# too-z/MultiModalPFN

Hardware: AMD Instinct MI355X
Metric: in-context rows/sec (support+query), PAD-UFES-20 shape, 1/2/4/8 MI355X (higher is better)
Workload: dtype f16

## Files before the change

### include/mmpfn_hip.h

```cpp
#ifndef MMPFN_HIP_H_
#define MMPFN_HIP_H_

#include <stdint.h>

#ifdef __cplusplus
extern "C" {
#endif

#define MMPFN_OK 0
#define MMPFN_ERR_INVALID (-1)
#define MMPFN_ERR_HIP (-2)
#define MMPFN_ERR_NAN (-3)
#define MMPFN_ERR_STATE (-4)
#define MMPFN_ERR_WEIGHT (-5)

#define MMPFN_PREC_F32 0
#define MMPFN_PREC_BF16 1
#define MMPFN_PREC_F32_MFMA 2
#define MMPFN_PREC_BF16_F8 3
#define MMPFN_PREC_BF16_F8E5 4
#define MMPFN_PREC_F16 5
#define MMPFN_PREC_F16_F8 6
#define MMPFN_PREC_F16_F8E5 7

// ... 30 lines not shown
const char* mmpfn_last_error(const mmpfn_ctx* ctx);
int mmpfn_set_stream(mmpfn_ctx* ctx, void* hip_stream);
const char* mmpfn_version(void);

int mmpfn_set_model(mmpfn_ctx* ctx, const mmpfn_model_desc* desc);
int mmpfn_load_weight(mmpfn_ctx* ctx, const char* name, const float* host_data, int64_t numel);
int mmpfn_finalize_weights(mmpfn_ctx* ctx);

int mmpfn_mixer_tokens(const mmpfn_ctx* ctx, int n_mod);
int mmpfn_mixer_forward(mmpfn_ctx* ctx, const float* image, int S, int n_mod, float* tokens, int precision);

int mmpfn_forward(mmpfn_ctx* ctx, const float* x, int S, int F, const float* tokens, int C, const float* y_train,
                  int N, const float* uniq, int U, const float* pos_rand, float* logits, int precision);

int mmpfn_set_full_last_layer(mmpfn_ctx* ctx, int on);

int mmpfn_embed(mmpfn_ctx* ctx, const float* x, int S, int F, const float* tokens, int C, const float* y_train, int N,
                const float* uniq, int U, const float* pos_rand, int precision);
int mmpfn_run_layers(mmpfn_ctx* ctx, int layer_begin, int layer_end);
int mmpfn_decode(mmpfn_ctx* ctx, float* logits);
int mmpfn_copy_state(mmpfn_ctx* ctx, float* out, int64_t capacity_elems);
int mmpfn_state_tokens(const mmpfn_ctx* ctx);

int mmpfn_aggregate(mmpfn_ctx* ctx, const float* logits, int M, int Q, int n_out, const int* perms, int n_cls,
                    float temperature, int average_before_softmax, const float* class_weights, float* probs);

#define MMPFN_BAR_MAX_BARS 8192
#define MMPFN_BAR_MAX_MEMBERS 1024
#define MMPFN_BAR_MAX_LEVELS 64
int mmpfn_bar_head(mmpfn_ctx* ctx, const float* logits, int M, int Q, int B, const unsigned char* cancel, int ldc,
// ... 71 lines not shown
```

### multimodalpfn_amd/_lib.py

```python

from __future__ import annotations

import ctypes
import os
from pathlib import Path

LIB_PATH = Path(__file__).resolve().parent / "libmmpfn_hip.so"

MMPFN_OK = 0
MMPFN_MAX_LANES = 8
MMPFN_ERR_INVALID = -1
MMPFN_ERR_HIP = -2
MMPFN_ERR_NAN = -3
MMPFN_ERR_STATE = -4
MMPFN_ERR_WEIGHT = -5
BAR_MAX_BARS, BAR_MAX_MEMBERS, BAR_MAX_LEVELS = 8192, 1024, 64
BAR_MAX_TARGETS, BAR_SCORE_ENDS = 64, 9

PREC_F32 = 0
PREC_BF16 = 1
PREC_F32_MFMA = 2
PREC_BF16_F8 = 3
PREC_BF16_F8E5 = 4
PREC_F16 = 5
# ... 83 lines not shown
    ("mmpfn_cache_free", None, [_vp, _vp]),
    ("mmpfn_kernel_timing", _i, [_vp, _i]),
    ("mmpfn_feature_attention", _i, [_vp, _i, _vp, _i, _i, _i]),
    ("mmpfn_feature_attention_ex", _i, [_vp, _i, _vp, _i, _i, _i, _i, _i]),
    ("mmpfn_item_attention_block", _i, [_vp, _i, _vp, _i, _i, _i, _i]),
    ("mmpfn_mlp_ln", _i, [_vp, _i, _vp, _i64, _i]),
    ("mmpfn_outproj_mlp_ln", _i, [_vp, _i, _vp, _vp, _i64, _i]),
    ("mmpfn_item_qkv", _i, [_vp, _i, _vp, _i, _i, _i, _i, _i, _i, _vp, _vp, _vp]),
    ("mmpfn_mgm", _i, [_vp, _vp, _i, _i, _vp, _i]),
    ("mmpfn_cap", _i, [_vp, _vp, _i, _i, _vp, _i]),
    ("mmpfn_kernel_timing_read", _i, [_vp, ctypes.POINTER(ctypes.c_double), ctypes.POINTER(ctypes.c_int64),
                                      ctypes.POINTER(ctypes.c_double)]),
    ("mmpfn_siphash24_rows", _i, [_vp, _i64, _i64, _vp]),
    ("mmpfn_set_parity_attention_min_keys", _i, [_i, _i]),
    ("mmpfn_set_full_last_layer", _i, [_vp, _i]),
    ("mmpfn_bar_head", _i, [_vp, _vp, _i, _i, _i, _vp, _i, _vp, _vp, _i, _f, _i, _vp, _vp, _vp, _vp, _vp, _i, _vp, _vp,
                            _vp, _vp]),
    ("mmpfn_bar_score", _i, [_vp, _vp, _i, _i, _f, _vp, _vp, _vp, _vp, _vp, _vp, _vp, _i, _vp, _vp, _vp, _vp, _vp]),
    ("mmpfn_bar_head_score", _i, [_vp, _vp, _i, _i, _i, _vp, _i, _vp, _vp, _i, _f, _i, _vp, _vp, _vp, _vp, _vp, _i, _vp,
                                  _vp, _vp, _vp, _vp, _vp, _vp, _vp, _vp, _i, _vp, _vp, _vp, _vp, _vp]),
]

MMPFN_ENC_VIT = 1
MMPFN_ENC_TEXT = 2


class EncDesc(ctypes.Structure):
    _fields_ = [
        ("kind", ctypes.c_int),
        ("dim", ctypes.c_int),
# ... 89 lines not shown
```

### multimodalpfn_amd/csrc/attention.hip

```cpp
#include <atomic>

#include "attn_item.h"
#include "common.h"
#include "kernels.h"

namespace mmpfn {

namespace {

constexpr int IA_KT = 64;

template <bool BF16>
struct IaLds {
  static constexpr int KROW = BF16 ? 80 : 144;
  static constexpr int VROW = BF16 ? 136 : 272;
  static constexpr int KBYTES = IA_KT * KROW;
  static constexpr int VBYTES = 32 * VROW;
  static constexpr int STAGE = KBYTES + VBYTES;
};

constexpr float IA_TAU = 8.0f;

template <int MODE, int NW>
__global__ __launch_bounds__(64 * NW) void attn_item_kernel(const AttnArgs p) {
// ... 696 lines not shown
      exact_rows(p, Kg, Vg, qrow, orow, qok[qb] && hh == 0, c);
      continue;
    }
    const float inv = 1.0f / ls;
    if (qok[qb]) {
#pragma unroll
      for (int gq = 0; gq < 4; ++gq)
        *(f32x4*)(orow + 8 * gq + 4 * hh) = f32x4{o[qb][4 * gq] * inv, o[qb][4 * gq + 1] * inv,
                                                  o[qb][4 * gq + 2] * inv, o[qb][4 * gq + 3] * inv};
    }
  }
}

}


namespace {
#ifndef X3_CHEAP_MIN_KEYS
#define X3_CHEAP_MIN_KEYS (-1)
#endif
#ifndef X3_CHEAP_FORM
#define X3_CHEAP_FORM 3
#endif
std::atomic<int> g_x3_cheap_min_keys{X3_CHEAP_MIN_KEYS};
std::atomic<int> g_x3_cheap_form{X3_CHEAP_FORM};

hipError_t launch_item_attention(const AttnLayerArgs& l, bool x3, hipStream_t st) {
  const int T = l.T, H = l.H, Npad = l.Npad, nk = l.nk, na = l.na, nb = l.nb, kvb = l.kvb;
  if (na + nb <= 0 || T <= 0) return hipSuccess;
  if (nk <= 0 || Npad % A2_KT != 0 || nk > Npad || H > 8 || H <= 0) return hipErrorInvalidValue;
  if (nb > 0 && (kvb < 0 || kvb >= H)) return hipErrorInvalidValue;
  if (l.qk_t == DType::F32 || l.o_t == DType::F32 || (l.qk_t == DType::F16 && l.o_t != DType::F16))
    return hipErrorInvalidValue;
  Attn2Args a;
  a.q = (const bf16*)l.q, a.k = (const bf16*)l.k, a.vt = (const bf16*)l.vt, a.o = (bf16*)l.out;
  a.S = l.S, a.H = H, a.Npad = Npad, a.nk = nk;
  a.a0 = l.a0, a.na = na, a.b0 = l.b0, a.nb = nb, a.kvb = nb > 0 ? kvb : -1;
  a.kv_bstride = l.kv_bstride > 0 ? l.kv_bstride : (int64_t)H * Npad * 32;
  a.q_prescaled = !x3 && l.q_prescaled ? 1 : 0;
  a.vt8 = (const unsigned char*)l.vt8, a.f8 = x3 ? 0 : l.f8;
  a.qk_f16 = (!x3 && l.qk_t == DType::F16) ? 1 : 0;
  a.o_f16 = (!x3 && l.o_t == DType::F16) ? 1 : 0;
  if (l.kv_bstride > 0 && (na > 0 || kvb != 0)) return hipErrorInvalidValue;
  const int qpb = x3 ? A3_QPB : ATTN_ITEM_QPB;
  int acc = 0;
  for (int g = 0; g < H; ++g) {
    a.tstart[g] = acc;
    const int cnt = na + (g == a.kvb ? H * nb : 0);
    acc += (cnt + qpb - 1) / qpb;
  }
  for (int g = H; g < 9; ++g) a.tstart[g] = acc;
  a.tasks_per_b = acc;
  a.nblocks = acc * T;
  if (a.nblocks == 0) return hipSuccess;
  if (x3) {
    const int mk = g_x3_cheap_min_keys.load(std::memory_order_relaxed);
    const int form = mk >= 0 && nk >= mk ? g_x3_cheap_form.load(std::memory_order_relaxed) : 0;
    if (form == 1) hipLaunchKernelGGL(attn_item3_kernel<1>, dim3(a.nblocks), dim3(256), 0, st, a);
    else if (form == 2) hipLaunchKernelGGL(attn_item3_kernel<2>, dim3(a.nblocks), dim3(256), 0, st, a);
    else if (form == 3) hipLaunchKernelGGL(attn_item3_kernel<3>, dim3(a.nblocks), dim3(256), 0, st, a);
    else hipLaunchKernelGGL(attn_item3_kernel<0>, dim3(a.nblocks), dim3(256), 0, st, a);
    return hipGetLastError();
  }
  return launch_attn_pipe(a, st);
}

}

// ... 55 lines not shown
```

### multimodalpfn_amd/csrc/attention_pipe.hip

```cpp
#include <type_traits>

#include "attn_item.h"
#include "common.h"
#include "kernels.h"
#include "lds_dma.h"

namespace mmpfn {

namespace {

#ifdef MMPFN_STAMPS
constexpr int AP_NST = 48;
__device__ unsigned long long g_ap_stamps[8 * 4 * AP_NST];
__device__ int g_ap_meta[4];
#define AP_STAMP(k)                                                                                     \
  do {                                                                                                  \
    const int sb_ = (int)blockIdx.x - (int)(gridDim.x / 2);                                            \
    if (sb_ >= 0 && sb_ < 8 && lane == 0) g_ap_stamps[(sb_ * 4 + wave) * AP_NST + (k)] = __builtin_amdgcn_s_memtime(); \
  } while (0)
#elif defined(MMPFN_STAMPS_ALL)
constexpr int AP_NST = 36, AP_MAXB = 8192;
__device__ unsigned long long g_ap_all[AP_MAXB * 4 * (AP_NST + 2)];
#define AP_STAMP(k)                                                                                     \
  do {                                                                                                  \
// ... 31 lines not shown
template <> struct P8<2> {
  static constexpr int FMT = 1, ETOP = 6, EMIN = -16, EMAX = 15;
  static constexpr float UFLOW = 0x1p-10f;
  static __device__ __forceinline__ s16x2 cvt(s16x2 old, float a, float b, float sc, bool hi) {
    return hi ? __builtin_amdgcn_cvt_scalef32_pk_bf8_f32(old, a, b, sc, true)
              : __builtin_amdgcn_cvt_scalef32_pk_bf8_f32(old, a, b, sc, false);
  }
};

constexpr int SG_VALU = 0x2, SG_MFMA = 0x8, SG_VMEM_READ = 0x20, SG_DS_READ = 0x100, SG_DS_WRITE = 0x200,
              SG_TRANS = 0x400;

#ifndef P4_DMA
#define P4_DMA 1
#endif
template <int F8, bool QF16, bool OF16>
__global__ __launch_bounds__(256, 2) void attn_pipe_kernel(const Attn2Args p) {
  typedef typename Op16<QF16>::t QT;
  typedef typename Op16<QF16>::x8 Q8;
  typedef typename Op16<OF16>::t OT;
  typedef typename Op16<OF16>::x4 O4;
  constexpr bool DMA = F8 == 0 && P4_DMA;
  constexpr int KROW = DMA ? 64 : 80;
  constexpr int VROW = F8 ? 80 : (DMA ? 128 : 144);
  constexpr int P4_SLOT_BYTES = 64 * KROW + 32 * VROW;
  __shared__ __attribute__((aligned(1024))) unsigned char ring[4 * P4_SLOT_BYTES];
  const int tid = threadIdx.x, lane = tid & 63;
  const int wave = __builtin_amdgcn_readfirstlane(tid >> 6);
  const int r = lane & 31, hh = lane >> 5;
  AP_STAMP(0);
#ifdef MMPFN_STAMPS_ALL
  if (lane == 0 && blockIdx.x < AP_MAXB) {
    const size_t b0 = ((size_t)blockIdx.x * 4 + wave) * (AP_NST + 2);
    g_ap_all[b0] = __builtin_amdgcn_s_getreg(4 | (31 << 11));
    g_ap_all[b0 + 1] = __builtin_amdgcn_s_getreg(20 | (31 << 11));
  }
#endif

  int b, g, chunk;
  {
    const int task = xcd_task(blockIdx.x, p.nblocks);
    b = task / p.tasks_per_b;
    const int rem = task - b * p.tasks_per_b;
    g = 0;
    int base = p.tstart[0];
#pragma unroll
    for (int h = 1; h < 9; ++h)
      if (h < p.H && p.tstart[h] <= rem) g = h, base = p.tstart[h];
    chunk = rem - base;
  }
  const int cnt = item_count(p, g);
  const int jw = chunk * P4_QPB + wave * P4_QPW;
  const bool active = jw < cnt;

  const int64_t kvoff = (int64_t)b * p.kv_bstride + (int64_t)g * p.Npad * 32;
  const QT* Kg = (const QT*)p.k + kvoff;
  const bf16* Vg = p.vt + kvoff;
  const unsigned char* Vg8 = p.vt8 + kvoff;
  const float c = kLog2e * 0.17677669529663687f;

  auto qrow_of = [&](int qb) __attribute__((always_inline)) { return item_query(p, g, cnt, jw + 32 * qb + r); };
  Q8 qf[P4_NCH][2];
#pragma unroll
  for (int qb = 0; qb < P4_NCH; ++qb) {
    const ItemQuery q = qrow_of(qb);
    const QT* qrow = (const QT*)p.q + (((int64_t)b * p.H + q.h) * p.S + q.s) * 32;
#pragma unroll
// ... 42 lines not shown
  };
  using VFrag = std::conditional_t<F8 != 0, i32x8, bf16x8[2][2]>;
  using PFrag = std::conditional_t<F8 != 0, i32x8, bf16x8[2][2]>;
  using VStage = std::conditional_t<F8 != 0, u32x2, u32x4>;
  auto readv = [&](VFrag& vf, const unsigned char* slot) __attribute__((always_inline)) {
    if constexpr (F8 != 0) {
      const u32x4 a = *(const u32x4*)(slot + vb), c = *(const u32x4*)(slot + vb + 16);
      vf = i32x8{(int)a.x, (int)a.y, (int)a.z, (int)a.w, (int)c.x, (int)c.y, (int)c.z, (int)c.w};
    } else {
#pragma unroll
      for (int u = 0; u < 2; ++u)
#pragma unroll
        for (int sp = 0; sp < 2; ++sp) vf[u][sp] = *(const bf16x8*)(slot + vro[u][sp]);
    }
  };
  const int krow = tid >> 2, kc = tid & 3, vd = tid >> 3, vc = tid & 7;
  const int kso = krow * 32 + kc * 8, vso = vd * p.Npad + vc * 8;
  const int kw = krow * KROW + 16 * (DMA ? kc ^ ((krow >> 2) & 3) : kc);
  const int vw = F8    ? VBASE + vd * VROW + 32 * (vc & 1) + 8 * (vc >> 1)
                 : DMA ? VBASE + vd * VROW + 16 * (vc ^ ((vd >> 1) & 7))
                       : VBASE + vd * VROW + 16 * vc;
  uint32_t kdo = 0, vdo = 0;
  if constexpr (DMA) {
    const int R = 16 * wave + (lane >> 2), d = 8 * wave + (lane >> 3);
    kdo = (uint32_t)(R * 32 + 8 * ((lane & 3) ^ ((R >> 2) & 3))) * 2;
    vdo = (uint32_t)(d * p.Npad + 8 * ((lane & 7) ^ ((d >> 1) & 7))) * 2;
  }
  const unsigned lds0 = (unsigned)(uintptr_t)(__attribute__((address_space(3))) void*)ring;
  auto dma = [&](int t, int slot) __attribute__((always_inline)) {
    lds_dma16(kdo, Kg + (int64_t)t * (P4_KT * 32), __builtin_amdgcn_readfirstlane(lds0 + slot * P4_SLOT_BYTES + wave * 1024));
    lds_dma16(vdo, Vg + t * P4_KT,
             __builtin_amdgcn_readfirstlane(lds0 + slot * P4_SLOT_BYTES + VBASE + wave * 1024));
  };
#ifndef P4_LEAD
#define P4_LEAD 2
#endif
  constexpr int LEAD = P4_LEAD;
  static_assert(LEAD == 1 || LEAD == 2, "staging lead");
  u32x4 rk[LEAD];
  VStage rv[LEAD];
  auto gload = [&](int t, u32x4& k, VStage& v) __attribute__((always_inline)) {
    k = *(const u32x4*)(Kg + (int64_t)t * (P4_KT * 32) + kso);
    if constexpr (F8 != 0) v = *(const u32x2*)(Vg8 + t * P4_KT + vso);
    else v = *(const u32x4*)(Vg + t * P4_KT + vso);
  };
  auto lstore = [&](unsigned char* slot, const u32x4& k, const VStage& v) __attribute__((always_inline)) {
    *(u32x4*)(slot + kw) = k;
    *(VStage*)(slot + vw) = v;
  };
  auto mask_pad = [&](u32x4& k, VStage& v) {
    const int k0 = nfull * P4_KT;
    if (k0 + krow >= p.nk) k = u32x4{0u, 0u, 0u, 0u};
    if constexpr (F8 != 0) {
      uint64_t e = __builtin_bit_cast(uint64_t, v);
#pragma unroll
      for (int j = 0; j < 8; ++j)
        if (k0 + vc * 8 + j >= p.nk) e &= ~((uint64_t)0xff << (8 * j));
      v = __builtin_bit_cast(u32x2, e);
    } else {
      bf16x8 e = __builtin_bit_cast(bf16x8, v);
#pragma unroll
      for (int j = 0; j < 8; ++j)
        if (k0 + vc * 8 + j >= p.nk) e[j] = (bf16)0.0f;
      v = __builtin_bit_cast(u32x4, e);
    }
// ... 159 lines not shown
    }
    __builtin_amdgcn_sched_group_barrier(SG_TRANS, P4_PIN == 2 ? 8 : 4, 0);
    __builtin_amdgcn_sched_group_barrier(SG_VALU, 16, 0);
    if (mem && !DMA) {
      __builtin_amdgcn_sched_group_barrier(SG_DS_WRITE, 2, 0);
      __builtin_amdgcn_sched_group_barrier(SG_VMEM_READ, 2, 0);
    }
#endif
  };

  if (ntiles > 0) {
    Q8 kf[2][2][2];
    VFrag vf[2];
    f32x16 sa[2], sb[2];
    PFrag pa, pz;
    {
      u32x4 rk1;
      VStage rv1;
      gload(tile_of(0), rk[0], rv[0]);
      gload(tile_of(min(1, ntiles - 1)), rk1, rv1);
      if constexpr (DMA) dma(tile_of(min(2, ntiles - 1)), 2);
      if (partial) mask_pad(rk[0], rv[0]);
      lstore(ring, rk[0], rv[0]);
      lstore(ring + P4_SLOT_BYTES, rk1, rv1);
    }
    if constexpr (!DMA) {
      gload(tile_of(min(2, ntiles - 1)), rk[0], rv[0]);
      if constexpr (LEAD == 2) gload(tile_of(min(3, ntiles - 1)), rk[1], rv[1]);
    }
    lds_barrier();
    AP_STAMP(2);
    if (!active) {
      if constexpr (DMA) {
        for (int t = 0; t < ntiles; ++t) {
          dma(tile_of(min(t + 3, ntiles - 1)), (t + 3) & 3);
          lds_barrier();
        }
        __builtin_amdgcn_s_waitcnt(0x0070);
        return;
      }
      for (int t = 0; t < ntiles; t += LEAD) {
        lstore(ring + ((t + 2) & 3) * P4_SLOT_BYTES, rk[0], rv[0]);
        gload(tile_of(min(t + 2 + LEAD, ntiles - 1)), rk[0], rv[0]);
        lds_barrier();
        if (LEAD == 2 && t + 1 < ntiles) {
          lstore(ring + ((t + 3) & 3) * P4_SLOT_BYTES, rk[LEAD - 1], rv[LEAD - 1]);
          gload(tile_of(min(t + 5, ntiles - 1)), rk[LEAD - 1], rv[LEAD - 1]);
// ... 2 lines not shown
      }
      return;
    }
    readk(kf[0], ring);
    if constexpr (F8 != 0) {
      vf[0] = i32x8{0, 0, 0, 0, 0, 0, 0, 0}, pz = vf[0];
    } else {
#pragma unroll
      for (int u = 0; u < 2; ++u)
#pragma unroll
        for (int sp = 0; sp < 2; ++sp)
#pragma unroll
          for (int j = 0; j < 8; ++j) vf[0][u][sp][j] = pz[u][sp][j] = (bf16)0.0f;
    }
    smm(sa, kf[0], 0);
    if constexpr (F8 != 0) {
      f32x16 s1[2];
      smm(s1, kf[0], 1);
      const int k0 = tile_of(0) * P4_KT;
#pragma unroll
      for (int qb = 0; qb < P4_NCH; ++qb) {
        const f32x16(&s)[2] = qb == 0 ? sa : s1;
        float m = -INFINITY;
#pragma unroll
        for (int u = 0; u < 2; ++u)
#pragma unroll
          for (int i = 0; i < 16; ++i)
            if (k0 + 32 * u + 16 * (i >> 3) + 8 * hh + (i & 7) < p.nk) m = fmaxf(m, s[u][i]);
        const auto sw = __builtin_amdgcn_permlane32_swap(__float_as_uint(m), __float_as_uint(m), false, false);
        m = fmaxf(__uint_as_float(sw[0]), __uint_as_float(sw[1]));
// ... 25 lines not shown
      pin_step(true);
      if constexpr (DMA) dma(tile_of(min(t + 3, ntiles - 1)), (L + 3) & 3);
      smm(sa, kf[B], 0);
      expc(pz, sb, 1);
      pv(0, pa, vf[B]);
      pin_step(false);
      lds_barrier();
#if defined(MMPFN_STAMPS) || defined(MMPFN_STAMPS_ALL)
      if (t < AP_NST - 6) AP_STAMP(3 + t);
#endif
    };
    using I0 = std::integral_constant<int, 0>;
    using I1 = std::integral_constant<int, 1>;
    using I2 = std::integral_constant<int, 2>;
    using I3 = std::integral_constant<int, 3>;
    int t = 0;
    for (; t + 4 <= ntiles; t += 4) {
      iter(I0{}, t);
      iter(I1{}, t + 1);
      iter(I2{}, t + 2);
      iter(I3{}, t + 3);
    }
    if (t < ntiles) iter(I0{}, t++);
    if (t < ntiles) iter(I1{}, t++);
    if (t < ntiles) iter(I2{}, t++);
    if (ntiles & 1) pv(1, pz, vf[1]);
    else pv(1, pz, vf[0]);
  }
  AP_STAMP(AP_NST - 3);

  if (!active) return;
  float mref[P4_NCH] = {0.f, 0.f};
  auto tile1 = [&](int t, bool first, bool ref) {
    const int k0 = t * P4_KT;
    Q8 kf[2][2];
    bf16x8 vf[2][2];
    loadk(kf, t);
    loadv(vf, t);
    const bool mask = k0 + P4_KT > p.nk;
    if (mask) {
// ... 71 lines not shown
    for (int gq = 0; gq < 4; ++gq) {
      O4 v;
#pragma unroll
      for (int e = 0; e < 4; ++e) v[e] = (OT)(o[qb][4 * gq + e] * inv);
      w[gq] = __builtin_bit_cast(u32x2, v);
    }
#pragma unroll
    for (int gg = 0; gg < 4; gg += 2) {
      const auto sx = __builtin_amdgcn_permlane32_swap(w[gg].x, w[gg + 1].x, false, false);
      const auto sy = __builtin_amdgcn_permlane32_swap(w[gg].y, w[gg + 1].y, false, false);
      const u32x4 st = hh == 0 ? u32x4{w[gg].x, w[gg].y, sx[1], sy[1]} : u32x4{sx[0], sy[0], w[gg + 1].x, w[gg + 1].y};
      if (q.ok) *(u32x4*)(orow + 8 * gg + 8 * hh) = st;
    }
  }
  AP_STAMP(AP_NST - 1);
}

}

namespace {
template <bool QF16, bool OF16>
hipError_t launch_pipe(const Attn2Args& a, hipStream_t st) {
  if (a.f8 == 1) {
    if (!a.vt8) return hipErrorInvalidValue;
    hipLaunchKernelGGL((attn_pipe_kernel<1, QF16, OF16>), dim3(a.nblocks), dim3(256), 0, st, a);
  } else if (a.f8 == 2) {
    if (!a.vt8) return hipErrorInvalidValue;
    hipLaunchKernelGGL((attn_pipe_kernel<2, QF16, OF16>), dim3(a.nblocks), dim3(256), 0, st, a);
  } else {
    hipLaunchKernelGGL((attn_pipe_kernel<0, QF16, OF16>), dim3(a.nblocks), dim3(256), 0, st, a);
// ... 6 lines not shown
extern "C" int mmpfn_dbg_attn_stamps(unsigned long long* stamps, int* meta) {
  hipError_t e = hipMemcpyFromSymbol(stamps, HIP_SYMBOL(g_ap_stamps), sizeof(g_ap_stamps));
  if (e == hipSuccess) e = hipMemcpyFromSymbol(meta, HIP_SYMBOL(g_ap_meta), sizeof(g_ap_meta));
  return (int)e;
}
#endif

#ifdef MMPFN_STAMPS_ALL
extern "C" int mmpfn_dbg_attn_stamps_all(unsigned long long* out, int nblocks) {
  const size_t n = (size_t)(nblocks < AP_MAXB ? nblocks : AP_MAXB) * 4 * (AP_NST + 2) * sizeof(unsigned long long);
  return (int)hipMemcpyFromSymbol(out, HIP_SYMBOL(g_ap_all), n);
}
#endif

hipError_t launch_attn_pipe(const Attn2Args& a, hipStream_t st) {
  if (a.qk_f16) return launch_pipe<true, true>(a, st);
  return a.o_f16 ? launch_pipe<false, true>(a, st) : launch_pipe<false, false>(a, st);
}

namespace {
__global__ void vt_fp8_kernel(const u32x4* __restrict__ in, u32x2* __restrict__ out, int64_t n8) {
  const int64_t i = (int64_t)blockIdx.x * blockDim.x + threadIdx.x;
  if (i >= n8) return;
  const bf16x8 v = __builtin_bit_cast(bf16x8, in[i]);
  float f[8];
#pragma unroll
  for (int j = 0; j < 8; ++j) f[j] = fminf(fmaxf((float)v[j], -448.f), 448.f);
  s16x2 lo = __builtin_amdgcn_cvt_scalef32_pk_fp8_f32(s16x2{0, 0}, f[0], f[1], 1.0f, false);
  lo = __builtin_amdgcn_cvt_scalef32_pk_fp8_f32(lo, f[2], f[3], 1.0f, true);
  s16x2 hi = __builtin_amdgcn_cvt_scalef32_pk_fp8_f32(s16x2{0, 0}, f[4], f[5], 1.0f, false);
// ... 16 lines not shown
```

### multimodalpfn_amd/csrc/attn_item.h

```cpp
#pragma once
#include "common.h"
#include "kernels.h"

namespace mmpfn {

struct Attn2Args {
  const __bf16* q;
  const __bf16* k;
  const __bf16* vt;
  __bf16* o;
  int S, H, Npad, nk;
  int a0, na;
  int b0, nb, kvb;
  int tasks_per_b, nblocks;
  int tstart[9];
  int64_t kv_bstride;
  int q_prescaled;
  const unsigned char* vt8;
  int f8;
  int qk_f16;
  int o_f16;
};
hipError_t launch_attn_pipe(const Attn2Args& a, hipStream_t st);

__device__ __forceinline__ int item_count(const Attn2Args& p, int g) { return p.na + (g == p.kvb ? p.H * p.nb : 0); }

struct ItemQuery {
  int h, s;
  bool ok;
};
// ... 45 lines not shown
```

### multimodalpfn_amd/csrc/capi.cpp

```cpp
#include <hip/hip_runtime.h>

#include <cmath>
#include <cstdlib>
#include <cstdio>
#include <cstring>
#include <map>
#include <string>
#include <utility>
#include <vector>

#include "../../include/mmpfn_hip.h"
#include "devbuf.h"
#include "kernels.h"
#include "weight_pack.h"

using namespace mmpfn;

namespace {

struct LayerW {
  Weight feat_qkv, feat_out, item_qkv, item_qtest, item_out, mlp1, mlp2;
  Weight feat_pack;
};

// ... 35 lines not shown
  std::string err;
  bool have_model = false, finalized = false;
  mmpfn_model_desc d{};
  std::map<std::string, std::vector<float>> host;

  ModelWeights w;

  DevBuf mx[8];
  DevBuf tap_v8;
  DevBuf tap_x16;
  std::vector<Lane> lanes;
  int cur = 0;
  mmpfn_cache* cache_out = nullptr;
  const mmpfn_cache* cache_in = nullptr;
  bool full_last = false;
  bool kt_on = false;
  std::vector<hipEvent_t> kt_pool;
  size_t kt_used = 0;
  double kt_flops = 0.0;
};

namespace {

#define HIPCHK(expr) HIPCHK_ON(ctx, expr)
#define GETW(var, name, n) GETW_ON(ctx, var, name, n)

bool mgm_f16_shape(const mmpfn_model_desc& d) { return (d.mgm_heads * d.nhid) % 256 == 0; }

int ensure_flag(mmpfn_ctx* ctx, DevBuf& b, hipStream_t st) {
  if (b.p) return MMPFN_OK;
// ... 383 lines not shown
  const int eb = pm.op_bytes();
  hipStream_t st = ctx->stream;
  void* O = ctx->ws_O.p;
  unsigned char* big = (unsigned char*)ctx->ws_big.p;
  void* Qi = big;
  void* Ki = big + (size_t)RM * E * eb;
  void* Vi = (unsigned char*)Ki + (size_t)TM * H * Npad * 32 * eb;
  RC(item_project(ctx, l, Xv, S, T, N, Npad, M, pm, last, ctx->cache_in != nullptr, Qi, Ki, Vi));
  if (ctx->cache_in) {
    const mmpfn_cache* cc = ctx->cache_in;
    const size_t kvl = (size_t)T * cc->Npad * 32 * eb;
    const size_t ccol = (size_t)c0 * cc->Npad * 32 * eb;
    const unsigned char* Kc = (const unsigned char*)cc->kv.p + (size_t)l * 2 * kvl + ccol;
    AttnLayerArgs a{Qi, Kc, Kc + kvl, O, S, TM, H, cc->Npad, cc->N};
    a.a0 = 0, a.na = 0, a.b0 = 0, a.nb = S, a.kvb = 0;
    a.kv_bstride = (int64_t)cc->Npad * 32;
    a.q_prescaled = pm.is16(), a.qk_t = pm.qk(), a.o_t = pm.attn_out();
    HIPCHK(launch_attn_layer(a, pm.base, st));
  } else {
    if (ctx->cache_out) {
      mmpfn_cache* cc = ctx->cache_out;
      const size_t blk = (size_t)Npad * 32 * eb, kvl = (size_t)T * blk;
      unsigned char* Kc = (unsigned char*)cc->kv.p + (size_t)l * 2 * kvl + c0 * blk;
      HIPCHK(hipMemcpy2DAsync(Kc, blk, Ki, (size_t)H * blk, blk, nc, hipMemcpyDeviceToDevice, st));
      HIPCHK(hipMemcpy2DAsync(Kc + kvl, blk, Vi, (size_t)H * blk, blk, nc, hipMemcpyDeviceToDevice, st));
    }
    if (last && Q == 0) return MMPFN_OK;
    AttnLayerArgs a{Qi, Ki, Vi, O, S, TM, H, Npad, N};
    a.a0 = 0, a.na = N, a.b0 = N, a.nb = Q, a.kvb = 0;
    if (last) a.na = N % ATTN_ITEM_QPB, a.a0 = N - a.na;
    a.q_prescaled = pm.is16(), a.qk_t = pm.qk(), a.o_t = pm.attn_out();
    hipEvent_t* ev = nullptr;
    if (pm.is16()) {
      if (ctx->kt_on && !last) {
        if (ctx->kt_used + 2 > ctx->kt_pool.size()) {
          for (int i = 0; i < 64; ++i) {
            hipEvent_t e;
            HIPCHK(hipEventCreate(&e));
            ctx->kt_pool.push_back(e);
          }
        }
        ev = &ctx->kt_pool[ctx->kt_used];
        ctx->kt_used += 2;
        ctx->kt_flops += 4.0 * TM * (double)(N + Q) * N * E;
      }
// ... 535 lines not shown
    }
  }
  if (bad) return fail(ctx, MMPFN_ERR_NAN, "There should be no NaNs in the encoded x and y (flag " + std::to_string(bad) + ")");
  return MMPFN_OK;
}

static int attn_tap_args(mmpfn_ctx* ctx, const void* q, const void* k, const void* vt, void* out, int S, int T, int H,
                         int Hmax, int Npad, int nk, int a0, int na, int b0, int nb, int kvb, AttnLayerArgs& a) {
  if (!ctx || !q || !k || !vt || !out) return MMPFN_ERR_INVALID;
  if (a0 < 0 || na < 0 || a0 + na > S || b0 < 0 || nb < 0 || b0 + nb > S || nk <= 0 || nk > Npad || Npad % 64 ||
      H <= 0 || H > Hmax || T <= 0 || kvb >= H)
    return fail(ctx, MMPFN_ERR_INVALID, "bad attention geometry");
  HIPCHK(hipSetDevice(ctx->device));
  a = AttnLayerArgs{q, k, vt, out, S, T, H, Npad, nk};
  a.a0 = a0, a.na = na, a.b0 = b0, a.nb = nb, a.kvb = kvb;
  return MMPFN_OK;
}

int mmpfn_item_attention(mmpfn_ctx* ctx, const void* q, const void* k, const void* vt, void* out, int S, int T, int H,
                         int Npad, int s0, int nq, int nk, int kvh, int precision) {
  AttnLayerArgs a;
  if (kvh < 0) RC(attn_tap_args(ctx, q, k, vt, out, S, T, H, INT32_MAX, Npad, nk, s0, nq, 0, 0, -1, a));
  else RC(attn_tap_args(ctx, q, k, vt, out, S, T, H, INT32_MAX, Npad, nk, 0, 0, s0, nq, kvh, a));
  if (precision != PREC_F32 && precision != PREC_BF16 && precision != PREC_F32_MFMA)
    return fail(ctx, MMPFN_ERR_INVALID, "bad precision (PREC_F32, PREC_BF16 or PREC_F32_MFMA; 16-bit / fp8 Q.K forms: "
                                        "mmpfn_item_attention_layer_ex)");
  HIPCHK(launch_attn_layer(a, precision, ctx->stream));
  return MMPFN_OK;
}

// ... 61 lines not shown
  if (ctx) {
    (void)hipSetDevice(ctx->device);
    (void)hipStreamSynchronize(ctx->stream);
  }
  delete cache;
}

int mmpfn_set_parity_attention_min_keys(int n, int form) { return mmpfn::set_x3_cheap_min_keys(n, form); }

int mmpfn_set_full_last_layer(mmpfn_ctx* ctx, int on) {
  if (!ctx) return MMPFN_ERR_INVALID;
  ctx->full_last = on != 0;
  return MMPFN_OK;
}

int mmpfn_kernel_timing(mmpfn_ctx* ctx, int enable) {
  if (!ctx) return MMPFN_ERR_INVALID;
  if (enable) ctx->kt_used = 0, ctx->kt_flops = 0.0;
  ctx->kt_on = enable != 0;
  return MMPFN_OK;
}

int mmpfn_kernel_timing_read(mmpfn_ctx* ctx, double* total_ms, int64_t* launches, double* flops) {
  if (!ctx || !total_ms || !launches || !flops) return MMPFN_ERR_INVALID;
  HIPCHK(hipSetDevice(ctx->device));
  double tot = 0.0;
  for (size_t i = 0; i + 1 < ctx->kt_used; i += 2) {
    HIPCHK(hipEventSynchronize(ctx->kt_pool[i + 1]));
    float ms = 0.f;
    HIPCHK(hipEventElapsedTime(&ms, ctx->kt_pool[i], ctx->kt_pool[i + 1]));
// ... 132 lines not shown
```

### multimodalpfn_amd/csrc/kernels.h

```cpp
#pragma once
#include <hip/hip_runtime.h>
#include <stdint.h>

#include "weight_pack.h"

namespace mmpfn {

enum Prec : int {
  PREC_F32 = 0,
  PREC_BF16 = 1,
  PREC_F32_MFMA = 2,
  PREC_BF16_F8 = 3,
  PREC_BF16_F8E5 = 4,
  PREC_F16 = 5,
  PREC_F16_F8 = 6,
  PREC_F16_F8E5 = 7
};
inline int base_prec(int p) {
  return p == PREC_BF16_F8 || p == PREC_BF16_F8E5 ? PREC_BF16 : p == PREC_F16_F8 || p == PREC_F16_F8E5 ? PREC_F16 : p;
}
inline int f8_of(int p) {
  return p == PREC_BF16_F8 || p == PREC_F16_F8 ? 1 : p == PREC_BF16_F8E5 || p == PREC_F16_F8E5 ? 2 : 0;
}
inline bool prec_ok(int p) { return p >= PREC_F32 && p <= PREC_F16_F8E5; }
// ... 86 lines not shown
hipError_t launch_attn(const AttnArgs& a, int batches, int prec, int waves_per_block, hipStream_t st);

struct AttnLayerArgs {
  const void* q;
  const void* k;
  const void* vt;
  void* out;
  int S, T, H, Npad, nk;
  int a0, na;
  int b0, nb, kvb;
  int64_t kv_bstride = 0;
  bool q_prescaled = false;
  const void* vt8 = nullptr;
  int f8 = 0;
  DType qk_t = DType::BF16, o_t = DType::BF16;
};
constexpr int ATTN_ITEM_QPB = 256;
hipError_t launch_attn_layer(const AttnLayerArgs& a, int base_prec, hipStream_t st);
hipError_t launch_vt_fp8(const void* vt, void* vt8, int64_t n, hipStream_t st);
int set_x3_cheap_min_keys(int n, int form);

struct SlotParams {
  int src;
  float fill;
  float lo, hi;
  float mean, sd;
  float scale;
};
hipError_t launch_encode_stats(const float* x , int S, int F, int N, int G, int fpg, float sigma,
                               SlotParams* slots, const float* y, int ny, float* ymean, hipStream_t st);
hipError_t launch_assemble(const float* x, int S, int F, int G, int fpg, int nf, const SlotParams* slots,
                           const float* w_enc , const float* posemb ,
                           const float* tok , int C, const float* y, int N, const float* uniq, int U,
// ... 80 lines not shown
```

### multimodalpfn_amd/engine.py

```python

from __future__ import annotations

import ctypes
import itertools
import os

import numpy as np
import torch

from multimodalpfn_amd import _lib
from multimodalpfn_amd.model.spec import CRITERION_PREFIX, ModelConfig, encoder_linear_name


def _ptr(t: torch.Tensor | None) -> int | None:
    return None if t is None else t.data_ptr()


def _count(t: torch.Tensor | None) -> int:
    return 0 if t is None else t.numel()


def model_desc(cfg: ModelConfig) -> _lib.ModelDesc:
    d = _lib.ModelDesc()
    d.emsize = cfg.emsize
# ... 38 lines not shown

_LANE_STREAMS: dict = {}


def _lane_stream(device: torch.device, k: int) -> torch.cuda.Stream:
    key = (str(device), k)
    st = _LANE_STREAMS.get(key)
    if st is None:
        st = _LANE_STREAMS[key] = torch.cuda.Stream(device)
    return st


DEFAULT_LANES = int(os.environ.get("MMPFN_LANES", "2"))
DEFAULT_BATCH = int(os.environ.get("MMPFN_BATCH", "1"))
DEFAULT_FULL_LAST_LAYER = os.environ.get("MMPFN_FULL_LAST_LAYER") == "1"
_DEBUG_SYNC = os.environ.get("MMPFN_DEBUG_SYNC") == "1"
_DEBUG_KEEP = os.environ.get("MMPFN_DEBUG_KEEP") == "1"
_KEEP: list = []
_SERIAL = itertools.count(1)


class HipEngine:

    def __init__(self, cfg: ModelConfig, state_dict: dict, device: torch.device):
        if not torch.cuda.is_available():
            raise RuntimeError("the MMPFN HIP engine needs a ROCm GPU (torch.cuda.is_available() is False)")
        self.lib = _lib.load_library()
        self.cfg = cfg
        self.device = torch.device(device)
        if self.device.type != "cuda":
# ... 14 lines not shown
            else:
                a = np.ascontiguousarray(t, dtype=np.float32)
            self._check(
                self.lib.mmpfn_load_weight(self.ctx, name.encode(), a.ctypes.data_as(ctypes.c_void_p), a.size),
                f"mmpfn_load_weight({name})",
            )
            names.add(name)
        if encoder_linear_name(cfg) not in names:
            raise _lib.EngineError(f"state_dict lacks {encoder_linear_name(cfg)}")
        self._check(self.lib.mmpfn_finalize_weights(self.ctx), "mmpfn_finalize_weights")
        self._pos_cache: dict[int, torch.Tensor] = {}
        self._streams: list = []
        self.lanes = DEFAULT_LANES
        self.batch = DEFAULT_BATCH
        self.full_last_layer = DEFAULT_FULL_LAST_LAYER
        self.refs = 1
        self.serial = next(_SERIAL)

    def _stream(self) -> int:
        return torch.cuda.current_stream(self.device).cuda_stream

    def _check(self, rc: int, what: str) -> None:
        _lib.check(self.lib, self.ctx, rc, what)

    def _bind_stream(self) -> None:
        self._check(self.lib.mmpfn_set_stream(self.ctx, ctypes.c_void_p(self._stream())), "mmpfn_set_stream")

    @property
    def full_last_layer(self) -> bool:
        return self._full_last_layer

    @full_last_layer.setter
    def full_last_layer(self, on: bool) -> None:
        self._check(self.lib.mmpfn_set_full_last_layer(self.ctx, int(bool(on))), "mmpfn_set_full_last_layer")
        self._full_last_layer = bool(on)

    def release(self) -> None:
        self.refs -= 1
        if self.refs <= 0:
            self.close()

    def close(self) -> None:
        if getattr(self, "ctx", None):
            self.lib.mmpfn_destroy(self.ctx)
            self.ctx = None

    def __del__(self):
        try:
            self.close()
        except Exception:
# ... 504 lines not shown
```

Measured before the change: 780,500.

## Pack small attention remainders into per-wave units sharing one block

A per-head query count can leave a small remainder (at most 64 queries) beyond whole 256-query tasks. Before, each such remainder got a full 256-thread block. Now these remainders become per-wave units, four of which share one block, and each wave stages its own K/V tiles by LDS-DMA into a private two-slot ring. This is meant to cut idle waves and wasted block launches in the item attention kernel. In exchange it adds a second pipeline path with complex waitcnt scheduling and a doubled LDS ring for the DMA variant, which could lower occupancy. The feature is on by default and can be turned off with an environment variable.

```diff
diff --git a/include/mmpfn_hip.h b/include/mmpfn_hip.h
--- a/include/mmpfn_hip.h
+++ b/include/mmpfn_hip.h
@@ -68,6 +68,10 @@
                   int N, const float* uniq, int U, const float* pos_rand, float* logits, int precision);
 
 int mmpfn_set_full_last_layer(mmpfn_ctx* ctx, int on);
+
+int mmpfn_set_attention_packing(mmpfn_ctx* ctx, int on);
+int mmpfn_attention_task_map(int na, int nb, int H, int T, int kvb, int packing, int* full_blocks, int* packed_blocks,
+                             int* units, int max_units);
 
 int mmpfn_embed(mmpfn_ctx* ctx, const float* x, int S, int F, const float* tokens, int C, const float* y_train, int N,
                 const float* uniq, int U, const float* pos_rand, int precision);
diff --git a/multimodalpfn_amd/_lib.py b/multimodalpfn_amd/_lib.py
--- a/multimodalpfn_amd/_lib.py
+++ b/multimodalpfn_amd/_lib.py
@@ -121,6 +121,8 @@
     ("mmpfn_siphash24_rows", _i, [_vp, _i64, _i64, _vp]),
     ("mmpfn_set_parity_attention_min_keys", _i, [_i, _i]),
     ("mmpfn_set_full_last_layer", _i, [_vp, _i]),
+    ("mmpfn_set_attention_packing", _i, [_vp, _i]),
+    ("mmpfn_attention_task_map", _i, [_i, _i, _i, _i, _i, _i, ctypes.POINTER(_i), ctypes.POINTER(_i), _vp, _i]),
     ("mmpfn_bar_head", _i, [_vp, _vp, _i, _i, _i, _vp, _i, _vp, _vp, _i, _f, _i, _vp, _vp, _vp, _vp, _vp, _i, _vp, _vp,
                             _vp, _vp]),
     ("mmpfn_bar_score", _i, [_vp, _vp, _i, _i, _f, _vp, _vp, _vp, _vp, _vp, _vp, _vp, _i, _vp, _vp, _vp, _vp, _vp]),
diff --git a/multimodalpfn_amd/csrc/attention.hip b/multimodalpfn_amd/csrc/attention.hip
--- a/multimodalpfn_amd/csrc/attention.hip
+++ b/multimodalpfn_amd/csrc/attention.hip
@@ -734,6 +734,25 @@
 
 }
 
+ItemTaskMap item_task_map(int na, int nb, int H, int T, int kvb, bool pack) {
+  ItemTaskMap m{};
+  int acc = 0;
+  for (int g = 0; g < H; ++g) {
+    m.tstart[g] = acc;
+    const int cnt = na + (g == kvb ? H * nb : 0), rem = cnt % ATTN_ITEM_QPB;
+    if (pack && rem >= 1 && rem <= ATTN_ITEM_UNIT) {
+      acc += cnt / ATTN_ITEM_QPB;
+      m.unit_heads |= (unsigned)g << (4 * m.upb++);
+    } else {
+      acc += (cnt + ATTN_ITEM_QPB - 1) / ATTN_ITEM_QPB;
+    }
+  }
+  for (int g = H; g < 9; ++g) m.tstart[g] = acc;
+  m.tasks_per_b = acc;
+  m.full_blocks = acc * T;
+  m.packed_blocks = T / 4 * m.upb + (T % 4 * m.upb + 3) / 4;
+  return m;
+}
 
 namespace {
 #ifndef X3_CHEAP_MIN_KEYS
@@ -762,16 +781,11 @@
   a.qk_f16 = (!x3 && l.qk_t == DType::F16) ? 1 : 0;
   a.o_f16 = (!x3 && l.o_t == DType::F16) ? 1 : 0;
   if (l.kv_bstride > 0 && (na > 0 || kvb != 0)) return hipErrorInvalidValue;
-  const int qpb = x3 ? A3_QPB : ATTN_ITEM_QPB;
-  int acc = 0;
-  for (int g = 0; g < H; ++g) {
-    a.tstart[g] = acc;
-    const int cnt = na + (g == a.kvb ? H * nb : 0);
-    acc += (cnt + qpb - 1) / qpb;
-  }
-  for (int g = H; g < 9; ++g) a.tstart[g] = acc;
-  a.tasks_per_b = acc;
-  a.nblocks = acc * T;
+  const ItemTaskMap m = item_task_map(na, nb, H, T, a.kvb, l.pack && !x3 && a.f8 == 0);
+  for (int g = 0; g < 9; ++g) a.tstart[g] = m.tstart[g];
+  a.tasks_per_b = m.tasks_per_b;
+  a.nblocks = m.full_blocks + m.packed_blocks;
+  a.ncol = T, a.upb = m.upb, a.unit_heads = m.unit_heads;
   if (a.nblocks == 0) return hipSuccess;
   if (x3) {
     const int mk = g_x3_cheap_min_keys.load(std::memory_order_relaxed);
diff --git a/multimodalpfn_amd/csrc/attention_pipe.hip b/multimodalpfn_amd/csrc/attention_pipe.hip
--- a/multimodalpfn_amd/csrc/attention_pipe.hip
+++ b/multimodalpfn_amd/csrc/attention_pipe.hip
@@ -69,19 +69,26 @@
 #ifndef P4_DMA
 #define P4_DMA 1
 #endif
-template <int F8, bool QF16, bool OF16>
-__global__ __launch_bounds__(256, 2) void attn_pipe_kernel(const Attn2Args p) {
+template <int F8> struct P4Lds {
+  static constexpr bool DMA = F8 == 0 && P4_DMA;
+  static constexpr int KROW = DMA ? 64 : 80;
+  static constexpr int VROW = F8 ? 80 : (DMA ? 128 : 144);
+  static constexpr int SLOT_BYTES = 64 * KROW + 32 * VROW;
+  static constexpr int BYTES = (DMA ? 8 : 4) * SLOT_BYTES;
+};
+
+template <int F8, bool QF16, bool OF16, bool PK>
+__device__ __forceinline__ void attn_pipe_block(const Attn2Args& p, unsigned char* ring0, int b, const int sub) {
   typedef typename Op16<QF16>::t QT;
   typedef typename Op16<QF16>::x8 Q8;
   typedef typename Op16<OF16>::t OT;
   typedef typename Op16<OF16>::x4 O4;
-  constexpr bool DMA = F8 == 0 && P4_DMA;
-  constexpr int KROW = DMA ? 64 : 80;
-  constexpr int VROW = F8 ? 80 : (DMA ? 128 : 144);
-  constexpr int P4_SLOT_BYTES = 64 * KROW + 32 * VROW;
-  __shared__ __attribute__((aligned(1024))) unsigned char ring[4 * P4_SLOT_BYTES];
+  constexpr bool DMA = P4Lds<F8>::DMA;
+  constexpr int KROW = P4Lds<F8>::KROW, VROW = P4Lds<F8>::VROW, P4_SLOT_BYTES = P4Lds<F8>::SLOT_BYTES;
+  static_assert(!PK || DMA, "packed blocks stage by LDS-DMA");
   const int tid = threadIdx.x, lane = tid & 63;
   const int wave = __builtin_amdgcn_readfirstlane(tid >> 6);
+  unsigned char* const ring = ring0 + (PK ? wave * (2 * P4_SLOT_BYTES) : 0);
   const int r = lane & 31, hh = lane >> 5;
   AP_STAMP(0);
 #ifdef MMPFN_STAMPS_ALL
@@ -92,11 +99,15 @@
   }
 #endif
 
-  int b, g, chunk;
-  {
-    const int task = xcd_task(blockIdx.x, p.nblocks);
-    b = task / p.tasks_per_b;
-    const int rem = task - b * p.tasks_per_b;
+  int g, chunk;
+  if constexpr (PK) {
+    const int unit = 4 * sub + wave;
+    if (unit >= p.upb * p.ncol) return;
+    b = unit / p.upb;
+    g = (p.unit_heads >> (4 * (unit - b * p.upb))) & 15;
+    chunk = 0;
+  } else {
+    const int rem = sub;
     g = 0;
     int base = p.tstart[0];
 #pragma unroll
@@ -105,7 +116,7 @@
     chunk = rem - base;
   }
   const int cnt = item_count(p, g);
-  const int jw = chunk * P4_QPB + wave * P4_QPW;
+  const int jw = PK ? cnt / P4_QPB * P4_QPB : chunk * P4_QPB + wave * P4_QPW;
   const bool active = jw < cnt;
 
   const int64_t kvoff = (int64_t)b * p.kv_bstride + (int64_t)g * p.Npad * 32;
@@ -178,15 +189,20 @@
         for (int sp = 0; sp < 2; ++sp) vf[u][sp] = *(const bf16x8*)(slot + vro[u][sp]);
     }
   };
-  const int krow = tid >> 2, kc = tid & 3, vd = tid >> 3, vc = tid & 7;
-  const int kso = krow * 32 + kc * 8, vso = vd * p.Npad + vc * 8;
-  const int kw = krow * KROW + 16 * (DMA ? kc ^ ((krow >> 2) & 3) : kc);
-  const int vw = F8    ? VBASE + vd * VROW + 32 * (vc & 1) + 8 * (vc >> 1)
-                 : DMA ? VBASE + vd * VROW + 16 * (vc ^ ((vd >> 1) & 7))
-                       : VBASE + vd * VROW + 16 * vc;
+  int krow, kc, vd, vc, kso, vso, kw, vw;
+  auto stage_as = [&](int id) __attribute__((always_inline)) {
+    krow = id >> 2, kc = id & 3, vd = id >> 3, vc = id & 7;
+    kso = krow * 32 + kc * 8, vso = vd * p.Npad + vc * 8;
+    kw = krow * KROW + 16 * (DMA ? kc ^ ((krow >> 2) & 3) : kc);
+    vw = F8    ? VBASE + vd * VROW + 32 * (vc & 1) + 8 * (vc >> 1)
+         : DMA ? VBASE + vd * VROW + 16 * (vc ^ ((vd >> 1) & 7))
+               : VBASE + vd * VROW + 16 * vc;
+  };
+  stage_as(tid);
   uint32_t kdo = 0, vdo = 0;
   if constexpr (DMA) {
-    const int R = 16 * wave + (lane >> 2), d = 8 * wave + (lane >> 3);
+    const int dw = PK ? 0 : wave;
+    const int R = 16 * dw + (lane >> 2), d = 8 * dw + (lane >> 3);
     kdo = (uint32_t)(R * 32 + 8 * ((lane & 3) ^ ((R >> 2) & 3))) * 2;
     vdo = (uint32_t)(d * p.Npad + 8 * ((lane & 7) ^ ((d >> 1) & 7))) * 2;
   }
@@ -195,6 +211,18 @@
     lds_dma16(kdo, Kg + (int64_t)t * (P4_KT * 32), __builtin_amdgcn_readfirstlane(lds0 + slot * P4_SLOT_BYTES + wave * 1024));
     lds_dma16(vdo, Vg + t * P4_KT,
              __builtin_amdgcn_readfirstlane(lds0 + slot * P4_SLOT_BYTES + VBASE + wave * 1024));
+  };
+  auto dma_k = [&](int t, int slot) __attribute__((always_inline)) {
+#pragma unroll
+    for (int w = 0; w < 4; ++w)
+      lds_dma16(kdo, Kg + (int64_t)t * (P4_KT * 32) + w * (16 * 32),
+                __builtin_amdgcn_readfirstlane(lds0 + slot * P4_SLOT_BYTES + w * 1024));
+  };
+  auto dma_v = [&](int t, int slot) __attribute__((always_inline)) {
+#pragma unroll
+    for (int w = 0; w < 4; ++w)
+      lds_dma16((w & 1) ? vdo ^ 64u : vdo, Vg + t * P4_KT + (int64_t)w * 8 * p.Npad,
+                __builtin_amdgcn_readfirstlane(lds0 + slot * P4_SLOT_BYTES + VBASE + w * 1024));
   };
 #ifndef P4_LEAD
 #define P4_LEAD 2
@@ -212,7 +240,7 @@
     *(u32x4*)(slot + kw) = k;
     *(VStage*)(slot + vw) = v;
   };
-  auto mask_pad = [&](u32x4& k, VStage& v) {
+  auto mask_pad = [&](u32x4& k, VStage& v) __attribute__((always_inline)) {
     const int k0 = nfull * P4_KT;
     if (k0 + krow >= p.nk) k = u32x4{0u, 0u, 0u, 0u};
     if constexpr (F8 != 0) {
@@ -402,7 +430,19 @@
     VFrag vf[2];
     f32x16 sa[2], sb[2];
     PFrag pa, pz;
-    {
+    if constexpr (PK) {
+      dma_k(tile_of(min(1, ntiles - 1)), 1);
+      dma_v(tile_of(min(1, ntiles - 1)), 1);
+#pragma unroll
+      for (int w = 0; w < 4; ++w) {
+        stage_as(64 * w + lane);
+        gload(tile_of(0), rk[0], rv[0]);
+        if (partial) mask_pad(rk[0], rv[0]);
+        lstore(ring, rk[0], rv[0]);
+      }
+      __builtin_amdgcn_s_waitcnt(0x0070);
+      __builtin_amdgcn_sched_barrier(0);
+    } else {
       u32x4 rk1;
       VStage rv1;
       gload(tile_of(0), rk[0], rv[0]);
@@ -416,9 +456,9 @@
       gload(tile_of(min(2, ntiles - 1)), rk[0], rv[0]);
       if constexpr (LEAD == 2) gload(tile_of(min(3, ntiles - 1)), rk[1], rv[1]);
     }
-    lds_barrier();
+    if constexpr (!PK) lds_barrier();
     AP_STAMP(2);
-    if (!active) {
+    if (!PK && !active) {
       if constexpr (DMA) {
         for (int t = 0; t < ntiles; ++t) {
           dma(tile_of(min(t + 3, ntiles - 1)), (t + 3) & 3);
@@ -451,6 +491,11 @@
           for (int j = 0; j < 8; ++j) vf[0][u][sp][j] = pz[u][sp][j] = (bf16)0.0f;
     }
     smm(sa, kf[0], 0);
+    if constexpr (PK) {
+      __builtin_amdgcn_s_waitcnt(0xC07F);
+      __builtin_amdgcn_sched_barrier(0);
+      dma_k(tile_of(min(2, ntiles - 1)), 0);
+    }
     if constexpr (F8 != 0) {
       f32x16 s1[2];
       smm(s1, kf[0], 1);
@@ -506,16 +551,44 @@
     using I1 = std::integral_constant<int, 1>;
     using I2 = std::integral_constant<int, 2>;
     using I3 = std::integral_constant<int, 3>;
+    auto iterp = [&](auto phc, int t) __attribute__((always_inline)) {
+      constexpr int A = decltype(phc)::value, B = A ^ 1;
+      readk(kf[B], ring + B * P4_SLOT_BYTES);
+      readv(vf[B], ring + A * P4_SLOT_BYTES);
+      smm(sb, kf[A], 1);
+      expc(pa, sa, 0);
+      pv(1, pz, vf[A]);
+      pin_step(true);
+      __builtin_amdgcn_s_waitcnt(0xC07F);
+      __builtin_amdgcn_sched_barrier(0);
+      dma_k(tile_of(min(t + 3, ntiles - 1)), B);
+      dma_v(tile_of(min(t + 2, ntiles - 1)), A);
+      smm(sa, kf[B], 0);
+      expc(pz, sb, 1);
+      pv(0, pa, vf[B]);
+      pin_step(false);
+      __builtin_amdgcn_s_waitcnt(0x0078);
+      __builtin_amdgcn_sched_barrier(0);
+    };
     int t = 0;
-    for (; t + 4 <= ntiles; t += 4) {
-      iter(I0{}, t);
-      iter(I1{}, t + 1);
-      iter(I2{}, t + 2);
-      iter(I3{}, t + 3);
-    }
-    if (t < ntiles) iter(I0{}, t++);
-    if (t < ntiles) iter(I1{}, t++);
-    if (t < ntiles) iter(I2{}, t++);
+    if constexpr (PK) {
+      for (; t + 2 <= ntiles; t += 2) {
+        iterp(I0{}, t);
+        iterp(I1{}, t + 1);
+      }
+      if (t < ntiles) iterp(I0{}, t++);
+      __builtin_amdgcn_s_waitcnt(0x0F70);
+    } else {
+      for (; t + 4 <= ntiles; t += 4) {
+        iter(I0{}, t);
+        iter(I1{}, t + 1);
+        iter(I2{}, t + 2);
+        iter(I3{}, t + 3);
+      }
+      if (t < ntiles) iter(I0{}, t++);
+      if (t < ntiles) iter(I1{}, t++);
+      if (t < ntiles) iter(I2{}, t++);
+    }
     if (ntiles & 1) pv(1, pz, vf[1]);
     else pv(1, pz, vf[0]);
   }
@@ -617,6 +690,26 @@
     }
   }
   AP_STAMP(AP_NST - 1);
+}
+
+template <int F8, bool QF16, bool OF16>
+__global__ __launch_bounds__(256, 2) void attn_pipe_kernel(const Attn2Args p) {
+  __shared__ __attribute__((aligned(1024))) unsigned char ring[P4Lds<F8>::BYTES];
+  const int task = xcd_task(blockIdx.x, p.nblocks);
+  if constexpr (P4Lds<F8>::DMA) {
+    const int gsz = 4 * p.tasks_per_b + p.upb;
+    const int grp = task / gsz, rg = task - grp * gsz;
+    const int npk = (min(4, p.ncol - 4 * grp) * p.upb + 3) >> 2;
+    if (rg < npk) {
+      attn_pipe_block<0, QF16, OF16, true>(p, ring, 0, grp * p.upb + rg);
+      return;
+    }
+    const int bg = (rg - npk) / p.tasks_per_b;
+    attn_pipe_block<F8, QF16, OF16, false>(p, ring, 4 * grp + bg, rg - npk - bg * p.tasks_per_b);
+  } else {
+    const int b = task / p.tasks_per_b;
+    attn_pipe_block<F8, QF16, OF16, false>(p, ring, b, task - b * p.tasks_per_b);
+  }
 }
 
 }
@@ -653,6 +746,7 @@
 #endif
 
 hipError_t launch_attn_pipe(const Attn2Args& a, hipStream_t st) {
+  if (a.upb && (a.f8 || !P4Lds<0>::DMA)) return hipErrorInvalidValue;
   if (a.qk_f16) return launch_pipe<true, true>(a, st);
   return a.o_f16 ? launch_pipe<false, true>(a, st) : launch_pipe<false, false>(a, st);
 }
diff --git a/multimodalpfn_amd/csrc/attn_item.h b/multimodalpfn_amd/csrc/attn_item.h
--- a/multimodalpfn_amd/csrc/attn_item.h
+++ b/multimodalpfn_amd/csrc/attn_item.h
@@ -14,6 +14,9 @@
   int b0, nb, kvb;
   int tasks_per_b, nblocks;
   int tstart[9];
+  int ncol;
+  int upb;
+  unsigned unit_heads;
   int64_t kv_bstride;
   int q_prescaled;
   const unsigned char* vt8;
diff --git a/multimodalpfn_amd/csrc/capi.cpp b/multimodalpfn_amd/csrc/capi.cpp
--- a/multimodalpfn_amd/csrc/capi.cpp
+++ b/multimodalpfn_amd/csrc/capi.cpp
@@ -73,6 +73,7 @@
   mmpfn_cache* cache_out = nullptr;
   const mmpfn_cache* cache_in = nullptr;
   bool full_last = false;
+  bool attn_pack = true;
   bool kt_on = false;
   std::vector<hipEvent_t> kt_pool;
   size_t kt_used = 0;
@@ -486,6 +487,7 @@
     const unsigned char* Kc = (const unsigned char*)cc->kv.p + (size_t)l * 2 * kvl + ccol;
     AttnLayerArgs a{Qi, Kc, Kc + kvl, O, S, TM, H, cc->Npad, cc->N};
     a.a0 = 0, a.na = 0, a.b0 = 0, a.nb = S, a.kvb = 0;
+    a.pack = ctx->attn_pack;
     a.kv_bstride = (int64_t)cc->Npad * 32;
     a.q_prescaled = pm.is16(), a.qk_t = pm.qk(), a.o_t = pm.attn_out();
     HIPCHK(launch_attn_layer(a, pm.base, st));
@@ -501,6 +503,7 @@
     AttnLayerArgs a{Qi, Ki, Vi, O, S, TM, H, Npad, N};
     a.a0 = 0, a.na = N, a.b0 = N, a.nb = Q, a.kvb = 0;
     if (last) a.na = N % ATTN_ITEM_QPB, a.a0 = N - a.na;
+    a.pack = ctx->attn_pack;
     a.q_prescaled = pm.is16(), a.qk_t = pm.qk(), a.o_t = pm.attn_out();
     hipEvent_t* ev = nullptr;
     if (pm.is16()) {
@@ -1066,6 +1069,7 @@
   HIPCHK(hipSetDevice(ctx->device));
   a = AttnLayerArgs{q, k, vt, out, S, T, H, Npad, nk};
   a.a0 = a0, a.na = na, a.b0 = b0, a.nb = nb, a.kvb = kvb;
+  a.pack = ctx->attn_pack;
   return MMPFN_OK;
 }
 
@@ -1157,6 +1161,28 @@
   return MMPFN_OK;
 }
 
+int mmpfn_set_attention_packing(mmpfn_ctx* ctx, int on) {
+  if (!ctx) return MMPFN_ERR_INVALID;
+  ctx->attn_pack = on != 0;
+  return MMPFN_OK;
+}
+
+int mmpfn_attention_task_map(int na, int nb, int H, int T, int kvb, int packing, int* full_blocks, int* packed_blocks,
+                             int* units, int max_units) {
+  if (na < 0 || nb < 0 || H <= 0 || H > 8 || T <= 0 || (nb > 0 && (kvb < 0 || kvb >= H)) || max_units < 0 ||
+      (max_units > 0 && !units))
+    return MMPFN_ERR_INVALID;
+  if (nb == 0) kvb = -1;
+  const mmpfn::ItemTaskMap m = mmpfn::item_task_map(na, nb, H, T, kvb, packing != 0);
+  if (full_blocks) *full_blocks = m.full_blocks;
+  if (packed_blocks) *packed_blocks = m.packed_blocks;
+  for (int u = 0; u < m.upb * T && u < max_units; ++u) {
+    const int g = (m.unit_heads >> (4 * (u % m.upb))) & 15, cnt = na + (g == kvb ? H * nb : 0);
+    units[3 * u] = u / m.upb, units[3 * u + 1] = g, units[3 * u + 2] = cnt / ATTN_ITEM_QPB * ATTN_ITEM_QPB;
+  }
+  return m.upb * T;
+}
+
 int mmpfn_kernel_timing(mmpfn_ctx* ctx, int enable) {
   if (!ctx) return MMPFN_ERR_INVALID;
   if (enable) ctx->kt_used = 0, ctx->kt_flops = 0.0;
diff --git a/multimodalpfn_amd/csrc/kernels.h b/multimodalpfn_amd/csrc/kernels.h
--- a/multimodalpfn_amd/csrc/kernels.h
+++ b/multimodalpfn_amd/csrc/kernels.h
@@ -124,9 +124,19 @@
   const void* vt8 = nullptr;
   int f8 = 0;
   DType qk_t = DType::BF16, o_t = DType::BF16;
+  bool pack = true;
 };
 constexpr int ATTN_ITEM_QPB = 256;
+constexpr int ATTN_ITEM_UNIT = 64;
 hipError_t launch_attn_layer(const AttnLayerArgs& a, int base_prec, hipStream_t st);
+struct ItemTaskMap {
+  int tstart[9];
+  int tasks_per_b;
+  int upb;
+  unsigned unit_heads;
+  int full_blocks, packed_blocks;
+};
+ItemTaskMap item_task_map(int na, int nb, int H, int T, int kvb, bool pack);
 hipError_t launch_vt_fp8(const void* vt, void* vt8, int64_t n, hipStream_t st);
 int set_x3_cheap_min_keys(int n, int form);
 
diff --git a/multimodalpfn_amd/engine.py b/multimodalpfn_amd/engine.py
--- a/multimodalpfn_amd/engine.py
+++ b/multimodalpfn_amd/engine.py
@@ -76,6 +76,7 @@
 DEFAULT_LANES = int(os.environ.get("MMPFN_LANES", "2"))
 DEFAULT_BATCH = int(os.environ.get("MMPFN_BATCH", "1"))
 DEFAULT_FULL_LAST_LAYER = os.environ.get("MMPFN_FULL_LAST_LAYER") == "1"
+DEFAULT_ATTENTION_PACKING = os.environ.get("MMPFN_ATTN_PACK") != "0"
 _DEBUG_SYNC = os.environ.get("MMPFN_DEBUG_SYNC") == "1"
 _DEBUG_KEEP = os.environ.get("MMPFN_DEBUG_KEEP") == "1"
 _KEEP: list = []
@@ -120,6 +121,7 @@
         self.lanes = DEFAULT_LANES
         self.batch = DEFAULT_BATCH
         self.full_last_layer = DEFAULT_FULL_LAST_LAYER
+        self.attention_packing = DEFAULT_ATTENTION_PACKING
         self.refs = 1
         self.serial = next(_SERIAL)
 
@@ -140,6 +142,15 @@
     def full_last_layer(self, on: bool) -> None:
         self._check(self.lib.mmpfn_set_full_last_layer(self.ctx, int(bool(on))), "mmpfn_set_full_last_layer")
         self._full_last_layer = bool(on)
+
+    @property
+    def attention_packing(self) -> bool:
+        return self._attention_packing
+
+    @attention_packing.setter
+    def attention_packing(self, on: bool) -> None:
+        self._check(self.lib.mmpfn_set_attention_packing(self.ctx, int(bool(on))), "mmpfn_set_attention_packing")
+        self._attention_packing = bool(on)
 
     def release(self) -> None:
         self.refs -= 1
```

Result: no change. 787,900 (median of 6 runs) (+1.0%).
